# TACC/GraviT

Hardware: AMD Instinct MI355X
Metric: Mrays/s (primary+shadow) at 1080p, 10M-tri scene (higher is better)
Workload: dtype f32; 1 GPU; soup-10000000: 10000000 random triangles (Philox seed 12345, half-extent 0.005), 1920x1080, eye (.5,.5,3)->(.5,.5,.5), fov 30deg, 1 point light at the eye, depth 1 (primary + 1 shadow ray), AO off; scheduler=image, 1 domain, harness=native, settle_frames=0, normal_mode=flat

## Files before the change

### gravit_amd/capi.py

```python
import ctypes as C
import os

import numpy as np

from .layouts import HIT_DTYPE, LIGHT_DTYPE, MATERIAL_DTYPE, RAY_DTYPE

HERE = os.path.dirname(os.path.abspath(__file__))
LIB_PATH = os.environ.get("GVT_HIP_LIB") or os.path.join(HERE, "libgvt_hip.so")

ABI_VERSION = 6

SYMBOLS = [
    "gvt_hip_init", "gvt_hip_set_stream", "gvt_hip_synchronize", "gvt_hip_last_error",
    "gvt_hip_mesh_create", "gvt_hip_mesh_destroy", "gvt_hip_trace_ex", "gvt_hip_mesh_get_info", "gvt_hip_mesh_get_normals", "gvt_hip_mesh_update_vertices",
    "gvt_hip_trace", "gvt_hip_intersect", "gvt_hip_occluded",
    "gvt_hip_queue_create", "gvt_hip_queue_destroy", "gvt_hip_queue_reserve", "gvt_hip_queue_clear", "gvt_hip_queue_size",
    "gvt_hip_queue_append", "gvt_hip_queue_append_flags", "gvt_hip_abi_version", "gvt_hip_queue_export", "gvt_hip_trace_queue", "gvt_hip_trace_queue_sink",
    "gvt_hip_camera_generate",
    "gvt_hip_camera_generate_tiled",
    "gvt_hip_camera_filter",
    "gvt_hip_top_create", "gvt_hip_top_destroy", "gvt_hip_top_order", "gvt_hip_top_update", "gvt_hip_shuffle", "gvt_hip_queue_sizes",
    "gvt_hip_fb_create", "gvt_hip_fb_destroy", "gvt_hip_fb_clear", "gvt_hip_fb_download", "gvt_hip_fb_device_ptr",
    "gvt_hip_fb_write_ppm_bytes",
    "gvt_hip_profile", "gvt_hip_stats_read", "gvt_hip_stats_reset", "gvt_hip_set_option", "gvt_hip_is_experiments_build", "gvt_hip_counters_peek", "gvt_hip_visit_stats", "gvt_hip_wide_visit_stats", "gvt_hip_mesh_download_nodes", "gvt_hip_mesh_download_wide", "gvt_hip_mesh_download_clusters", "gvt_hip_mesh_upload_nodes", "gvt_hip_marked_visit_stats", "gvt_hip_image_frame",
# ... 8 lines not shown
    "gvt_hip_volume_create_typed", "gvt_hip_volume_update_samples_typed", "gvt_hip_volume_get_voxel_type",
]


class GvtHipError(RuntimeError):
    pass


class MeshInfo(C.Structure):
    _fields_ = [("n_tris", C.c_uint64), ("n_verts", C.c_uint64), ("n_nodes", C.c_uint64), ("n_leaves", C.c_uint64),
                ("bbox_lo", C.c_float * 3), ("bbox_hi", C.c_float * 3), ("build_ms", C.c_float), ("max_leaf", C.c_uint32),
                ("packet", C.c_uint32), ("bytes_nodes", C.c_uint64), ("bytes_tris", C.c_uint64), ("sah_inner", C.c_float), ("pad", C.c_float)]


class CameraPod(C.Structure):
    _fields_ = [("eye", C.c_float * 3), ("focus", C.c_float * 3), ("up", C.c_float * 3), ("fov", C.c_float), ("width", C.c_int32),
                ("height", C.c_int32), ("samples", C.c_int32), ("depth", C.c_int32), ("jitter_window_size", C.c_float)]


class FrameStats(C.Structure):
    _fields_ = [("rounds", C.c_uint64), ("chains", C.c_uint64), ("host_syncs", C.c_uint64), ("rays_sent", C.c_uint64),
                ("rays_closest", C.c_uint64), ("rays_any", C.c_uint64), ("packets_bailed", C.c_uint64), ("bytes_sent", C.c_uint64),
                ("ms_chain", C.c_double), ("ms_announce", C.c_double), ("ms_payload", C.c_double), ("ms_composite", C.c_double), ("ms_host_wait", C.c_double),
                ("exchanges", C.c_uint64), ("rays_inline", C.c_uint64)]

    def as_dict(self):
        return {k: getattr(self, k) for k, _ in self._fields_}


class VolumeInfo(C.Structure):
    _fields_ = [("box_lo", C.c_float * 3), ("box_hi", C.c_float * 3), ("dt", C.c_float), ("value_min", C.c_float), ("value_max", C.c_float),
                ("blocks", C.c_int32 * 3), ("pad", C.c_float), ("n_blocks", C.c_uint64), ("n_blocks_empty", C.c_uint64),
                ("samples_marched", C.c_uint64), ("samples_gathered", C.c_uint64)]

    def as_dict(self):
        return {k: (list(getattr(self, k)) if k in ("box_lo", "box_hi", "blocks") else getattr(self, k)) for k, _ in self._fields_ if k != "pad"}


RAY_OPAQUE, RAY_BOUNDARY, RAY_EXTERNAL_BOUNDARY = 0x2, 0x4, 0x10
RAY_SIDES = 0x20
VOLUME_MAX_SURFACES, VOLUME_MAX_LIGHTS = 16, 8
VOLUME_OPAQUE_A = 0.99
VOLUME_DEVICE, VOLUME_NO_SKIP = 1, 2
VOXEL_F32, VOXEL_U8, VOXEL_I16, VOXEL_U16 = 0, 1, 2, 3
VOXEL_TYPES = {"float32": VOXEL_F32, "uint8": VOXEL_U8, "int16": VOXEL_I16, "uint16": VOXEL_U16}

FRAME_BSP, FRAME_NO_COMPOSITE, FRAME_FULL_REDUCE, FRAME_IMAGE = 1, 2, 4, 8
# ... 113 lines not shown
```

### gravit_amd/csrc/api.hip

```cpp
#include <atomic>
#include <chrono>
#include <cmath>
#include <cstdlib>
#include <condition_variable>
#include <functional>
#include <mutex>
#include <new>
#include <thread>

#include "gvt_internal.h"

size_t trav_spill_ints_per_thread();
int trav_block_threads();
void abi_pool_destroy(void *);

static thread_local std::string g_err;
static Ctx g_default_ctx;
static thread_local Ctx *tl_ctx = nullptr;
#define g_ctx (gctx())
Ctx &gctx() { return tl_ctx ? *tl_ctx : g_default_ctx; }

void set_error(const char *fmt, ...) {
  char buf[1024];
  va_list ap;
// ... 191 lines not shown
extern "C" int gvt_hip_stats_reset(void) {
  if (ensure_init()) return GVT_HIP_ERR_NODEVICE;
  drain_events();
  g_ctx.stats = gvt_hip_stats{};
  return 0;
}

namespace {
struct KnobDef { const char *name; int Knobs::*field; int lo, hi; bool shipped; };
const KnobDef g_knobs[] = {
  { "skip_known", &Knobs::skip_known, 0, 1, true },           { "frame_timing", &Knobs::frame_timing, 0, 1, true },
  { "term_sink", &Knobs::term_sink, 0, 1, true },
  { "sort_rays", &Knobs::sort_rays, 0, 1, true },             { "leaf_max", &Knobs::leaf_max, 1, 4, true },
  { "long_steps", &Knobs::long_steps, 0, 1 << 20, true },     { "small_rays", &Knobs::small_rays, 0, 1 << 30, true },
  { "finish_rays", &Knobs::finish_rays, 0, 1 << 30, true },   { "round_room_mb", &Knobs::round_room_mb, 0, 1 << 30, true },
  { "abi_lanes", &Knobs::abi_lanes_n, 0, 8, true },           { "abi_chunk", &Knobs::abi_chunk, 16384, 1 << 30, true },
  { "inject_fail_tick", &Knobs::inject_fail_tick, -1, 1 << 30, true },
  { "long_min_rays", &Knobs::long_min_rays, 0, 1 << 30, true }, { "long_auto", &Knobs::long_auto, 0, 1, true },
  { "finish_auto", &Knobs::finish_auto, 0, 1, true },
  { "payload_overlap_kb", &Knobs::payload_overlap_kb, 0, 1 << 30, true },
  { "packet", &Knobs::packet, 0, 2, true },                   { "packet_sah_max", &Knobs::packet_sah_max, 0, 1 << 30, true },
  { "packet_min_rays", &Knobs::packet_min_rays, 0, 1 << 30, true },
  { "shadow_order", &Knobs::shadow_order, 0, 1, true },       { "shadow_order_min_rays", &Knobs::shadow_order_min_rays, 0, 1 << 30, true },
  { "xcd_stripes", &Knobs::xcd_stripes, 0, 1, true },

  { "inline_kb", &Knobs::inline_kb, 0, 1024, true },          { "comm_cus", &Knobs::comm_cus, 0, 128, true },
  { "comm_stream", &Knobs::comm_stream, 0, 1, true },         { "spec_ticks", &Knobs::spec_ticks, 0, 1, true },
  { "finish_clusters", &Knobs::finish_clusters, 0, 1, true }, { "hop_local", &Knobs::hop_local, 0, 3, true },
  { "blocks_per_cu", &Knobs::blocks_per_cu, 1, 8, false },    { "blocks_per_cu_closest", &Knobs::blocks_per_cu_closest, 0, 8, false },
  { "refill_min", &Knobs::refill_min, 1, 64, false },         { "inner_min", &Knobs::inner_min, 1, 64, false },
  { "share", &Knobs::share, 0, 1, false },                    { "share_min_rays", &Knobs::share_min_rays, 0, 1 << 30, false },
  { "sort_gather", &Knobs::sort_gather, 0, 1, false },        { "sort_bits", &Knobs::sort_bits, 8, 32, false },
  { "long_steps_drain", &Knobs::long_steps_drain, 0, 1 << 20, false }, { "long_save", &Knobs::long_save, 0, 1, false },
  { "lean_frame", &Knobs::lean_frame, 0, 1, false },          { "report_poll", &Knobs::report_poll, 0, 1, false },
  { "first_round_async", &Knobs::first_round_async, 0, 1, false }, { "wave_single", &Knobs::wave_single, 0, 1, false },
  { "shadow_direct", &Knobs::shadow_direct, 0, 1, false },    { "top_ordered", &Knobs::top_ordered, 0, 1, false },
  { "top_lds", &Knobs::top_lds, 0, 1, false },                { "camera_tile", &Knobs::camera_tile, 0, 8, false },
  { "abi_pipe_min", &Knobs::abi_pipe_min, 0, 1 << 30, false },
  { "shadow_cls_lo", &Knobs::shadow_cls_lo, 0, 255, false },  { "shadow_cls_shift", &Knobs::shadow_cls_shift, 0, 6, false },
};
}

extern "C" int gvt_hip_set_option(const char *name, int value) {
  if (!name) { set_error("set_option: null name"); return GVT_HIP_ERR_INVALID; }
  if (!std::strcmp(name, "defaults")) { static_cast<Knobs &>(g_ctx) = Knobs{}; return 0; }
  for (const KnobDef &k : g_knobs) {
    if (std::strcmp(name, k.name)) continue;
// ... 616 lines not shown
```

### gravit_amd/csrc/domain.hip

```cpp
#include <dlfcn.h>
#include <rccl/rccl.h>

#include <atomic>
#include <condition_variable>
#include <memory>
#include <mutex>

#include <chrono>
#include <thread>

#include "gvt_internal.h"

int shuffle_async(gvt_hip_top *T, gvt_hip_queue *q_in, size_t n_ub, const int *from_arr, int from, gvt_hip_queue *const *queues, const uint8_t *keep_mask,
                  gvt_hip_fb *fb, unsigned *d_overflow, const void *d_qdesc);
int shuffle_exact(gvt_hip_top *T, gvt_hip_queue *q_in, const int *from_arr, int from, gvt_hip_queue *const *queues, gvt_hip_fb *fb);
int camera_one_instance_async(gvt_hip_top *T, const gvt_hip_camera *cam, int tile, gvt_hip_queue *q, gvt_hip_fb *fb, unsigned *d_overflow, unsigned *d_moved_count, unsigned *row_rays);
int camera_filter_async(gvt_hip_top *T, const gvt_hip_camera *cam, int tile, gvt_hip_queue *const *queues, const uint8_t *keep_mask, unsigned *d_overflow,
                        size_t first, size_t count, bool rect = false, unsigned *row_rays = nullptr);
size_t camera_instance_bound(gvt_hip_top *T, const gvt_hip_camera *cam, int tile, size_t inst);

namespace {
struct Rccl {
  void *lib = nullptr;
  ncclResult_t (*GetUniqueId)(ncclUniqueId *) = nullptr;
// ... 716 lines not shown
  size_t inl_bytes = 0, msg_ints = 0;
  double tick_us[8] = { 0 }; uint64_t tick_n[8] = { 0 }; double comp_us = 0;
  uint64_t n_spec_enqueued = 0, n_spec_valid = 0, n_exchanges = 0;
  size_t spec_recent_rays = 0;
  bool sizes_exact = true;
  bool spec_enqueued_last = false;
  unsigned *d_spec = nullptr;
  WaveSeg *d_spec_segs = nullptr;
  bool layout_agreed = false;
  int *d_hs = nullptr, *h_hs = nullptr;
  unsigned *d_overflow = nullptr;
  std::vector<void *> send_buf, recv_buf;
  std::vector<size_t> send_cap, recv_cap;
  hipEvent_t ev_compute = nullptr, ev_report = nullptr, ev_pack = nullptr, ev_recv = nullptr, ev_comm = nullptr;
  hipEvent_t ev_chain0 = nullptr, ev_ann0 = nullptr, ev_pay0 = nullptr, ev_comp0 = nullptr;
  bool chain_timed = false, payload_timed = false;
  uint64_t last_local_pending = 0;
  std::vector<size_t> present;
  int long_cur = 0;
  uint64_t frame_no = 0;
  int fin_choice = -1;
  int fin_limit = 0;
  int hop_now = 0;
  unsigned cam_row_rays = 0;
  bool fin_eligible = false;
  unsigned fin_probe = 0;
  double fin_best[6] = { 1e30, 1e30, 1e30, 1e30, 1e30, 1e30 };
  int fin_n[6] = { 0, 0, 0, 0, 0, 0 };
  bool surfaces = false;
};

extern "C" void gvt_hip_tracer_destroy(gvt_hip_tracer *R) {
  if (!R) return;
  if (getenv("GVT_HIP_SPEC_TRACE") && R->n_exchanges)
    fprintf(stderr, "[tracer rank %d] %llu announce exchanges, speculative part enqueued behind %llu, valid %llu\n", R->rank, (unsigned long long)R->n_exchanges,
            (unsigned long long)R->n_spec_enqueued, (unsigned long long)R->n_spec_valid);
  if (getenv("GVT_HIP_SPEC_TRACE") && R->tick_n[0]) {
    fprintf(stderr, "[tracer rank %d] mean us from frame start / previous announce to the announce of tick:", R->rank);
    for (int k = 0; k < 8 && R->tick_n[k]; k++) fprintf(stderr, " %d: %.1f", k, R->tick_us[k] / (double)R->tick_n[k]);
    fprintf(stderr, "; last announce to frame end %.1f\n", R->comp_us / (double)R->tick_n[0]);
  }
  if (gctx().ready) hipStreamSynchronize(gctx().stream);
  if (R->comm && !R->comm->dead) hipStreamSynchronize(R->comm->stream);
  for (auto q : R->queues) gvt_hip_queue_destroy(q);
  gvt_hip_queue_destroy(R->q_moved);
  hipFree(R->d_insts); hipFree(R->d_round); hipHostFree(R->h_round); hipFree(R->d_count_ptr); hipFree(R->d_owner);
// ... 211 lines not shown
  R->sizes_exact = false;
  for (int k = 0; k < n_seg; k++) {
    gvt_hip_queue *q = R->queues[R->h_segs[k].inst];
    R->h_segs[k].planes = q->d_planes; R->h_segs[k].cap = q->cap;
  }
  hipStream_t st = C.stream;
  for (size_t i = 0; i < nI; i++) {
    gvt_hip_queue *Q = R->queues[i];
    R->h_qdesc[i].planes = Q->d_planes; R->h_qdesc[i].cap = Q->cap; R->h_qdesc[i].count = Q->d_count; R->h_qdesc[i].keep = 1u;
  }
  for (size_t k = (size_t)n_seg; k < (nI ? nI : 1); k++) std::memset(&R->h_segs[k], 0, sizeof(WaveSeg));
  if ((rc = round_tables_upload(R, st))) return rc;
  int *d_from = (int *)scratch_get(SCR_OUT_FROM, sizeof(int) * bound);
  if (!d_from) return GVT_HIP_ERR_DEVICE;
  TraceParams P{};
  P.normal_mode = R->normal_mode; P.seed = 0; P.n_lights = nL; P.update_in_place = 0; P.carried_rng = 1;
  P.sink = TermSink{};
  if (C.term_sink) {
    P.sink.top = R->top->dev(); P.sink.from = -1;
    P.sink.fb = R->fb->d_rgba; P.sink.n_pix = (unsigned)(R->fb->w * R->fb->h);
  }
  P.hop = R->hop_now == 1 ? 1 : R->hop_now == 2 ? 2 : 0;
  P.hop_owner = R->world > 1 ? R->d_owner : nullptr; P.hop_rank = R->rank;
  WaveSet W{ R->d_segs, R->d_insts, n_seg, (int)nI };
  if (C.finish_rays > 0 && N <= (size_t)C.finish_rays && P.sink.fb && !count_on_device && !exact) R->fin_eligible = true;
  if (R->fin_limit > 0 && N <= (size_t)R->fin_limit && P.sink.fb && !count_on_device && !exact) {
    if ((rc = finish_round(W, N, P, R->lights.data(), R->d_qdesc, R->d_owner, R->world > 1 ? R->rank : -1, R->d_overflow, R->d_count_ptr, R->d_mask))) return rc;
    if (chains) (*chains)++;
    return 0;
  }
  WaveSingle one{};
  if (n_seg == 1 && R->meshes[R->h_segs[0].inst] && C.wave_single && !P.hop) {
    const int i0 = R->h_segs[0].inst;
    one.planes = make_planes(R->h_segs[0].planes, R->h_segs[0].cap);
    if (nI == 1) one.planes.p5 = nullptr;
    one.mesh = R->meshes[i0]; one.inst = i0;
    one.coherent = (fresh_from_camera && C.camera_tile == 8) ? 1 : 0;
    one.row_rays = one.coherent ? R->cam_row_rays : 0u;
    one.n_dev = count_on_device ? R->queues[i0]->d_count : nullptr;
    one.pass0_begun = pass0_begun ? 1 : 0;
    std::memcpy(one.minv.m, R->minv.data() + 16 * (size_t)i0, 64);
    std::memcpy(one.normi.n, R->normi.data() + 9 * (size_t)i0, 36);
  }
  const bool single = one.mesh != nullptr;
  ChainOpts O;
  O.d_count_ptr = R->d_count_ptr; O.d_mask = R->d_mask; O.n_inst = (int)nI;
// ... 226 lines not shown
    if ((R->frame_no & 2047u) == 0 || (R->fin_choice >= 0 && !((allowed >> R->fin_choice) & 1u))) {
      R->fin_choice = -1;
      for (int v = 0; v < 6; v++) { R->fin_n[v] = 0; R->fin_best[v] = 1e30; }
    }
    if (R->fin_choice >= 0) fin_variant = R->fin_choice;
    else {
      int pick = fin_variant;
      for (int k = 0; k < n_allowed; k++) if (R->fin_n[route_list[k]] < R->fin_n[pick]) pick = route_list[k];
      fin_variant = pick;
    }
  }
  R->fin_limit = (fin_variant & 1) ? C.finish_rays : 0;
  R->hop_now = fin_variant >> 1;
  R->fin_eligible = false;
  struct LongOverride { Ctx &C; ~LongOverride() { C.long_steps_override = 0; } } long_override{ C };
  C.long_steps_override = (C.long_auto && C.long_steps > 0 && R->long_cur > C.long_steps) ? R->long_cur : 0;
  const bool one_shot = nI == 1 && R->world == 1 && C.term_sink && C.wave_single && R->meshes[0] && C.first_round_async;
  const bool lean = one_shot && C.lean_frame && R->fb->w == R->cam.width && R->fb->h == R->cam.height;
  for (size_t i = 0; i < nI; i++) R->queues[i]->size = 0;
  R->q_moved->size = 0;
  R->sizes_exact = true; R->spec_enqueued_last = false;
  R->cam_row_rays = 0u;
  bool first_on_device = false;
  if (!lean) {
    if ((rc = gvt_hip_fb_clear(R->fb))) return rc;
    k_zero_totals<<<(unsigned)std::max<size_t>(1, (nI + 255) / 256), 256, 0, st>>>(C.d_counters, R->d_overflow, R->fb->w, R->fb->h, R->d_count_ptr, (int)nI);
  }
  if (one_shot) {
    const size_t n_cam = (size_t)R->cam.width * R->cam.height * R->cam.samples * R->cam.samples;
    const int passes0 = R->cam.depth > 1 ? R->cam.depth : 1;
    if ((rc = queue_reserve(R->queues[0], n_cam * (size_t)(1 + (int)R->lights.size() * passes0)))) return rc;
    if (lean) { if ((rc = camera_one_instance_async(R->top, &R->cam, C.camera_tile, R->queues[0], R->fb, R->d_overflow, R->q_moved->d_count, &R->cam_row_rays))) return rc; }
    else if ((rc = camera_filter_async(R->top, &R->cam, C.camera_tile, R->queues.data(), nullptr, R->d_overflow, 0, 0, false, &R->cam_row_rays))) return rc;
    R->present[0] = n_cam;
    R->queues[0]->size = n_cam;
    if ((rc = local_chain(R, nullptr, &S.chains, true, true, lean, lean))) return rc;
    if ((rc = round_report(R, false, &S.host_syncs, lean))) return rc;
  } else if (image_split) {
    const size_t n_cam = (size_t)R->cam.width * R->cam.height * R->cam.samples * R->cam.samples;
    const size_t portion = n_cam / (size_t)R->world, first = (size_t)R->rank * portion;
    const size_t count = (R->rank + 1 == R->world) ? n_cam - first : portion;
    for (size_t i = 0; i < nI; i++) if ((rc = queue_reserve(R->queues[i], count))) return rc;
    if ((rc = camera_filter_async(R->top, &R->cam, C.camera_tile, R->queues.data(), nullptr, R->d_overflow, first, count))) return rc;
    std::fill(R->owned.begin(), R->owned.end(), (uint8_t)1);
    R->world = 1;
    if ((rc = round_report(R, false, &S.host_syncs))) return rc;
// ... 281 lines not shown
    R->fin_n[fin_variant]++;
    R->fin_probe++;
    bool once = true;
    double lead = 1e30;
    for (int k = 0; k < n_allowed; k++) { once = once && R->fin_n[route_list[k]] >= 1; lead = std::min(lead, R->fin_best[route_list[k]]); }
    if (once) for (int k = 0; k < n_allowed; k++) if (R->fin_best[route_list[k]] > 1.3 * lead) R->fin_n[route_list[k]] = std::max(R->fin_n[route_list[k]], 3);
    bool all = true;
    int best = route_list[0];
    for (int k = 0; k < n_allowed; k++) {
      all = all && R->fin_n[route_list[k]] >= 3;
      if (R->fin_best[route_list[k]] < R->fin_best[best] || (R->fin_best[route_list[k]] == R->fin_best[best] && route_list[k] > best)) best = route_list[k];
    }
    if (all) {
      R->fin_choice = best;
      if (getenv("GVT_HIP_ROUTE_TRACE")) {
        fprintf(stderr, "[tracer] frame %llu: route settled -- k_finish %d, hops %s; fastest frame per route timed, ms:", (unsigned long long)R->frame_no, best & 1,
                (best >> 1) == 0 ? "never" : (best >> 1) == 1 ? "early" : "always");
        for (int k = 0; k < n_allowed; k++) fprintf(stderr, " [k_finish %d hops %d] %.3f", route_list[k] & 1, route_list[k] >> 1, R->fin_best[route_list[k]]);
        fprintf(stderr, "\n");
      }
    }
  }
  R->frame_no++;
  if (out) *out = S;
  return 0;
}
```

### gravit_amd/csrc/gvt_internal.h

```cpp
#pragma once
#include <hip/hip_runtime.h>

#include <cstdarg>
#include <cstdio>
#include <cstring>
#include <string>
#include <vector>

#include "gvt_device.h"

enum KernelClass { KC_CLOSEST = 0, KC_ANY, KC_SHADE, KC_CONVERT, KC_SHUFFLE, KC_CAMERA, KC_BUILD, KC_SORT, KC_LONG, KC_COUNT };

struct PendingEvent {
  hipEvent_t a, b;
  int cls;
};

#define SHADOW_CLASSES 8
static_assert(CW_SHADOW_CLS + SHADOW_CLASSES <= CW_PEEK, "the class counts are read through gvt_hip_counters_peek");
static_assert(CW_SHADOW_CLS + SHADOW_CLASSES <= CW_COUNT && CW_PEEK <= CW_COUNT, "every named counter word lies inside the allocation");

enum ScratchSlot {
  SCR_GENERAL,
  SCR_SHADOW,
// ... 13 lines not shown
  SCR_VOL_RANGES,
  SCR_BUILD,
  SCR_HOP,
  SCRATCH_COUNT
};
struct Knobs {
  int blocks_per_cu = 4;
  int blocks_per_cu_closest = 5;
  int refill_min = 16;
  int inner_min = 32;
  int share = 1;
  int share_min_rays = 131072;
  int sort_rays = 0;
  int sort_gather = 0;
  int sort_bits = 20;
  int long_steps = 96;
  int long_steps_drain = 0;
  int long_save = 1;
  int long_min_rays = 65536;
  int packet = 1;
  int shadow_order = 1;
  int shadow_cls_lo = 24, shadow_cls_shift = 3;
  int xcd_stripes = 1;
  int shadow_order_min_rays = 262144;
  int packet_min_rays = 524288;
  int packet_sah_max = 128;
  int round_room_mb = 16384;
  int finish_rays = 32768;
  int finish_auto = 1;
  int small_rays = 4096;
  int abi_lanes_n = 4;
  int abi_chunk = 262144;
  int abi_pipe_min = 131072;
  int lean_frame = 1;
  int skip_known = 0;
  int long_auto = 1;
  int payload_overlap_kb = 1024;
  int inline_kb = 16;
  int comm_cus = 0;
  int hop_local = 1;
  int finish_clusters = 1;
  int spec_ticks = 1;
  int comm_stream = 0;
  int frame_timing = 0;
  int inject_fail_tick = -1;
  int report_poll = 1;
  int first_round_async = 1;
  int wave_single = 1;
  int shadow_direct = 1;
  int term_sink = 1;
  int camera_tile = 8;
  int top_ordered = 1;
  int top_lds = 1;
  int leaf_max = 2;
};

struct Ctx : Knobs {
  bool ready = false;
  int device = -1;
  hipStream_t own_stream = nullptr;
  hipStream_t stream = nullptr;
  int profile = 0;
  int long_steps_override = 0;
  std::vector<PendingEvent> pending;
  std::vector<hipEvent_t> event_pool;
  gvt_hip_stats stats{};
  int n_cu = 256;
  bool shadow_order_denied = false;
  int cu_reserved = 0;
  int trav_blocks = 0;
  int *d_spill = nullptr;
  unsigned *d_counters = nullptr;
  unsigned *h_pinned = nullptr;
  void *scratch[SCRATCH_COUNT] = { nullptr };
  size_t scratch_bytes[SCRATCH_COUNT] = { 0 };
  std::vector<unsigned char> lights_cached;
  const void *lights_cached_dst = nullptr;
  gvt_hip_queue *abi_qin = nullptr, *abi_qout = nullptr;
  std::vector<Ctx *> abi_lanes;
  void *abi_pool = nullptr;
};
Ctx &gctx();
void set_error(const char *fmt, ...);
int ensure_init();
inline bool staging_queues(Ctx &C) {
  if (!C.abi_qin) { C.abi_qin = gvt_hip_queue_create(0); C.abi_qout = gvt_hip_queue_create(0); }
  return C.abi_qin && C.abi_qout;
}
void *scratch_get(ScratchSlot slot, size_t bytes);
void scratch_release(ScratchSlot slot);
// ... 78 lines not shown
  unsigned long long cap;
  unsigned *count;
  unsigned keep;
};

struct TermSink {
  TopDev top;
  int from;
  float *fb;
  unsigned n_pix;
};
struct TraceParams {
  Mat4 m, minv;
  Mat3 normi;
  int normal_mode;
  uint32_t seed;
  int n_lights;
  TermSink sink;
  int update_in_place;
  int carried_rng;
  int hop;
  const int *hop_owner;
  int hop_rank;
};

struct MeshView {
  const float4 *slots;
  const unsigned *slot_of;
  const float *verts;
  const int *tris;
  const float *normals;
  const float *vcolors;
  const gvt_hip_material *materials;
  unsigned n_mat;
  const int *face_mat;
  gvt_hip_material mat;
};

struct WaveSeg {
  float4 *planes;
  unsigned long long cap;
  unsigned begin, n;
  int inst, pad;
};
struct WaveInst {
  Mat4 minv;
// ... 67 lines not shown
```

### gravit_amd/csrc/shade.inc

```
__device__ inline V3 light_contribution(const gvt_hip_light &L, V3 hit, V3 samplePos) {
  V3 c = ld3(L.color);
  if (L.type == GVT_HIP_LIGHT_AMBIENT) return c;
  V3 p = (L.type == GVT_HIP_LIGHT_AREA) ? samplePos : ld3(L.position);
  float distance = 1.f / len3(sub3(p, hit));
  distance = (distance > 1.f) ? 1.f : distance;
  return scl3(c, distance);
}

__device__ inline V3 area_light_position(const gvt_hip_light &L, uint32_t &seed) {
  V3 v = ld3(L.normal), u, w;
  if (v.x == 0.f && v.y == 1.f && v.z == 0.f) {
    u = mk3(1, 0, 0); w = mk3(0, 0, 1);
  } else {
    const V3 up = mk3(0, 1, 0);
    u.x = up.y * v.z - v.y * up.z; u.y = up.z * v.x - v.z * up.x; u.z = up.x * v.y - v.x * up.y;
    w.x = v.y * u.z - u.y * v.z; w.y = v.z * u.x - u.z * v.x; w.z = v.x * u.y - u.x * v.y;
  }
  float xLocation = (float)(((double)gvt_fastrand_lcg(seed, 0, 1) - 0.5) * (double)L.width);
  float zLocation = (float)(((double)gvt_fastrand_lcg(seed, 0, 1) - 0.5) * (double)L.height);
  float xCoord = xLocation * u.x + zLocation * w.x;
  float yCoord = xLocation * u.y + zLocation * w.y;
  float zCoord = xLocation * u.z + zLocation * w.z;
  return mk3(L.position[0] + xCoord, L.position[1] + yCoord, L.position[2] + zCoord);
}
// ... 123 lines not shown
  const gvt_hip_hit *hits;
  int first_pass;
  int carried_rng;
  RayPlanes out; unsigned *out_count;
  RayPlanes shadow; unsigned *shadow_count;
  unsigned *next_idx; unsigned *next_count;
  const gvt_hip_light *lights;
  Mat3 normi;
  int normal_mode, n_lights;
  uint32_t seed;
  unsigned *zero_word;
  TermSink sink;
  int update_in_place;
  const unsigned *n_dev;
  WaveSet W;
  const int *hop_inst;
  int *out_from;
  int *shadow_inst;
  unsigned shadow_stride;
  const unsigned char *steps;
  unsigned *cls_cnt;
  unsigned cls_stride;
  int cls_lo, cls_shift;
};

__device__ __forceinline__ unsigned shadow_class(int steps, int lo, int shift) {
  const int c = (steps - lo) >> shift;
  return (unsigned)(c < 0 ? 0 : (c > SHADOW_CLASSES - 1 ? SHADOW_CLASSES - 1 : c));
}

#define SHADE_BLOCK 512
template <bool MULTI, bool LEAN = false>
__global__ __launch_bounds__(SHADE_BLOCK, 4) void k_shade(ShadeArgs A, MeshView M1) {
  __shared__ unsigned sh_alloc[2 * (2 + 64)];
  __shared__ unsigned sh_cls[2 * SHADOW_CLASSES];
  for (int k = threadIdx.x; k < 2 * (2 + 64); k += SHADE_BLOCK) sh_alloc[k] = 0u;
  if (threadIdx.x < 2 * SHADOW_CLASSES) sh_cls[threadIdx.x] = 0u;
  __syncthreads();
  const unsigned j = blockIdx.x * blockDim.x + threadIdx.x;
  if (j == 0 && A.zero_word) *A.zero_word = 0u;
  const unsigned n = A.n_dev ? *A.n_dev : A.n;
  const bool in_range = j < n;
  __shared__ unsigned sh_wcls[SHADE_BLOCK / 64];
  if (!MULTI && A.cls_cnt) {
    int st = in_range ? (int)A.steps[j] : 0;
    for (int o = 32; o >= 1; o >>= 1) st = max(st, __shfl_xor(st, o));
    if (lane_id() == 0) sh_wcls[threadIdx.x >> 6] = shadow_class(st, A.cls_lo, A.cls_shift);
// ... 91 lines not shown
        s.c = c; s.t = r.t;
        s.id = r.id; s.depth = r.depth; s.w = r.w; s.type = 1;
        s.rng = 0u;
        s.km[0] = 0u; s.km[1] = 0u; s.km[2] = 0u;
      }
    }
    if (A.shadow_stride) {
      if (j < A.shadow_stride) {
        const unsigned slot = (unsigned)li * A.shadow_stride + j;
        A.shadow_inst[slot] = emit ? (MULTI ? inst : 0) : -1;
        if (emit) store_ray(A.shadow, slot, s);
      }
    } else if (!MULTI && A.cls_cnt) {
      const unsigned cls = (unsigned)__builtin_amdgcn_readfirstlane((int)sh_wcls[threadIdx.x >> 6]);
      const unsigned long long mask = ballot64(emit);
      unsigned woff = 0;
      if (mask) {
        if ((int)lane_id() == __ffsll((long long)mask) - 1) woff = atomicAdd(&sh_cls[cls], (unsigned)__popcll(mask));
        woff = (unsigned)__builtin_amdgcn_readlane((int)woff, __ffsll((long long)mask) - 1);
      }
      __syncthreads();
      if (threadIdx.x < SHADOW_CLASSES && sh_cls[threadIdx.x]) sh_cls[SHADOW_CLASSES + threadIdx.x] = atomicAdd(&A.cls_cnt[threadIdx.x], sh_cls[threadIdx.x]);
      __syncthreads();
      if (emit) store_ray(A.shadow, cls * A.cls_stride + sh_cls[SHADOW_CLASSES + cls] + woff + lanes_below(mask), s);
    } else {
      const unsigned slot = block_alloc(A.shadow_count, emit, &sh_alloc[2 * (2 + li)]);
      if (emit) { store_ray(A.shadow, slot, s); if (MULTI) A.shadow_inst[slot] = inst; }
    }
  }
  if (!LEAN && shaded) {
    const int ndepth = r.depth - 1;
    const float p = 1.f - gvt_fastrand01(g_seed);
    if (ndepth > 0 && r.w > p) {
      r.type = 2;
      const float multiplier = 1.0f - 16.0f * GVT_FLT_EPSILON;
      const float t_secondary = multiplier * r.t;
      r.o = add3(r.o, scl3(r.d, t_secondary));
      const V3 nd = cos_weighted_dir(N, g_seed);
      r.d = nd;
      r.w = r.w * dot3(nd, N);
      r.depth = ndepth;
      r.km[0] = 0u; r.km[1] = 0u; r.km[2] = 0u;
      bounce = true;
    }
    if (bounce || A.update_in_place) {
      r.rng = g_seed;
      store_ray(in, i, r);
    }
  }
  if (!LEAN) {
// ... 5 lines not shown
```

### gravit_amd/csrc/trace.hip

```cpp
#include "gvt_internal.h"

#ifndef TRAV_BLOCK
#define TRAV_BLOCK 256
#endif
#define TRAV_WAVES_PER_BLOCK (TRAV_BLOCK / 64)
#ifndef TRAV_STACK
#define TRAV_STACK 24
#endif
#ifndef KT_BLOCKS_CLOSEST
#define KT_BLOCKS_CLOSEST 5
#endif
#ifndef RETIRE_BATCH
#define RETIRE_BATCH 1
#endif
#ifndef KT_BLOCKS_ANY
#define KT_BLOCKS_ANY 4
#endif
#define TRAV_SPILL 128

namespace {

struct Trav {
  const BvhNode *__restrict__ nodes;
  const float4 *__restrict__ tris;
// ... 193 lines not shown
    ProfScope ps(KC_CLOSEST);
    LongQ LP{ d_long, c + CW_LONG, nullptr, 0u, 0, 0 };
    if constexpr (MULTI) k_packet_multi<<<blocks_for(n), 256, 0, st>>>(S.W, (unsigned)n, n_dev, tnear, d_hits, LP, c + CW_PACKETS);
    else k_packet<false><<<blocks_for(n), 256, 0, st>>>(S.q, (unsigned)n, n_dev, S.minv, S.T, tnear, d_hits, nullptr, none, nullptr, TermSink{}, LP, nullptr, nullptr, nullptr, c + CW_PACKETS);
    k_long_closest<XFORM, MULTI><<<tail_grid, 256, 0, st>>>(S.q, d_long, c + CW_LONG, S.minv, S.T, tnear, d_hits, c + CW_LONG_WORK, S.W);
  } else if (mode == BY_WAVES) {
    ProfScope ps(KC_CLOSEST);
    k_long_seed<<<blocks_for(n), 256, 0, st>>>(d_long, c + CW_LONG, idx, (unsigned)n, n_dev);
    k_long_closest<XFORM, MULTI><<<wave_grid(n), 256, 0, st>>>(S.q, d_long, c + CW_LONG, S.minv, S.T, tnear, d_hits, c + CW_LONG_WORK, S.W, nullptr, later_pass ? S.hop : nullptr);
  } else {
    {
      ProfScope ps(KC_CLOSEST);
      launch_trace<false, XFORM, 0, MULTI>(trav_grid2(n, true), st, S.q, idx, (unsigned)n, S.minv, S.T, tnear, d_hits, nullptr, none, nullptr, c + CW_WORK, C.d_spill,
                                           C.refill_min, C.inner_min, n_dev, C.share, (unsigned)C.share_min_rays, S.sink, LQ, S.MS, MULTI ? XCD_STRIPES_OFF : stripe_arg(S.row));
    }
    if (LQ.steps) {
      ProfScope ps(KC_LONG);
      k_long_closest<XFORM, MULTI><<<tail_grid, 256, 0, st>>>(S.q, LQ.recs, LQ.count, S.minv, S.T, tnear, d_hits, c + CW_LONG_WORK, S.W, LQ.stk, S.hop);
    }
  }
}

template <bool MULTI>
static void any_step(StepMode mode, const TraceSrc &S, const unsigned *idx, size_t grid_rays, unsigned n, const unsigned *n_dev, RayPlanes out, unsigned *out_count) {
  Ctx &C = gctx();
  unsigned *c = C.d_counters;
  ProfScope ps(KC_ANY);
  if (mode == BY_WAVES) k_wave_any<MULTI><<<wave_grid(grid_rays), 256, 0, C.stream>>>(S.q, c + CW_SHADOW, S.minv, S.T, GVT_RAY_EPSILON, out, out_count, c + CW_WORK, S.sink, S.MS);
  else launch_trace<true, true, 1, MULTI>(trav_grid2(grid_rays), C.stream, S.q, idx, n, S.minv, S.T, GVT_RAY_EPSILON, nullptr, nullptr, out, out_count, c + CW_WORK, C.d_spill,
                                          C.refill_min, C.inner_min, n_dev, C.share, (unsigned)C.share_min_rays, S.sink, LongQ{}, S.MS, MULTI ? XCD_STRIPES_OFF : stripe_arg(S.row));
}

static ShadeArgs shade_args(const ChainBufs &B, const unsigned *idx, size_t n, int pass, const unsigned *n_dev, unsigned *next, unsigned *c_next, RayPlanes outp,
                            unsigned *out_count, const TraceParams &P) {
  unsigned *c = gctx().d_counters;
  ShadeArgs A{};
  A.idx = idx; A.n = (unsigned)n; A.hits = B.hits; A.first_pass = (pass == 0); A.carried_rng = 1; A.out = outp; A.out_count = out_count;
  A.shadow = B.shadow; A.shadow_count = c + CW_SHADOW; A.next_idx = next; A.next_count = c_next; A.lights = B.lights; A.normi = P.normi; A.normal_mode = P.normal_mode;
  A.n_lights = P.n_lights; A.seed = P.seed; A.zero_word = c + CW_WORK; A.sink = P.sink; A.n_dev = n_dev;
  return A;
}

template <bool MULTI>
static void shade_step(const ShadeArgs &A, const MeshView &mv, bool lean = false) {
  ProfScope ps(KC_SHADE);
  if (lean) k_shade<MULTI, true><<<blocks_for(A.n, SHADE_BLOCK), SHADE_BLOCK, 0, gctx().stream>>>(A, mv);
  else k_shade<MULTI><<<blocks_for(A.n, SHADE_BLOCK), SHADE_BLOCK, 0, gctx().stream>>>(A, mv);
}

int launch_closest(gvt_hip_mesh *M, RayPlanes q, const unsigned *idx, size_t n, bool xform, const Mat4 &minv, float tnear,
// ... 199 lines not shown
  Ctx &C = gctx();
  unsigned *c = C.d_counters;
  gvt_hip_mesh *M = W1.mesh;
  const size_t n = K.n;
  const int nL = K.P.n_lights;
  const bool have4 = M->d_nodes4 != nullptr, by_class = K.B.steps != nullptr;
  if (C.sort_rays && p.pass > 0 && n >= 8192 && have4)
    if (int rc = sort_ray_list(M, W1.planes, &p.idx, n, n, W1.minv, p.n_dev)) return rc;
  TraceSrc S{};
  S.q = W1.planes; S.minv = W1.minv; S.T = Trav{ M->d_nodes, M->d_tri, M->d_nodes4 };
  S.row = (W1.coherent && p.pass == 0 && !p.idx) ? W1.row_rays : 0u;
  LongQ LQ{};
  if (K.use_long && have4) LQ = long_queue(K.d_long, n);
  LQ.steps_out = K.B.steps;
  const bool small1 = K.small && have4;
  const bool pkt = walks_packets(C, M, n) && W1.coherent && p.pass == 0 && have4 && !small1;
  const bool pkt_any = pkt && C.packet == 2;
  closest_step<true, false>(pkt ? BY_PACKETS : small1 ? BY_WAVES : BY_LANES, S, p.idx, n, p.n_dev, GVT_RAY_EPSILON, K.B.hits, LQ, K.d_long);
  ShadeArgs A = shade_args(K.B, p.idx, n, p.pass, p.n_dev, p.next, p.c_next, K.outp, K.out->d_count, K.P);
  A.in = W1.planes; A.normi = W1.normi; A.sink.from = W1.inst;
  if (pkt_any) { A.shadow_inst = K.d_shadow_inst; A.shadow_stride = (unsigned)n; }
  A.steps = K.B.steps; A.cls_cnt = by_class ? c + CW_SHADOW_CLS : nullptr; A.cls_stride = (unsigned)cls_stride; A.cls_lo = C.shadow_cls_lo; A.cls_shift = C.shadow_cls_shift;
  const bool lean_shade = W1.coherent && p.pass == 0 && K.passes == 1 && K.P.sink.fb && K.P.sink.top.n_inst == 1 && nL >= 1 && plain_lambert(M) && no_area_light(K.lights_host, nL);
  shade_step<false>(A, mesh_view(M), lean_shade);
  if (!nL) return 0;
  TraceSrc SA = S;
  SA.q = K.B.shadow; SA.sink = A.sink; SA.row = 0u;
  if (pkt_any) return any_packets(K, SA);
  if (by_class) { SA.MS.cls_cnt = c + CW_SHADOW_CLS; SA.MS.cls_stride = (unsigned)cls_stride; SA.MS.cls_total = c + CW_SHADOW; }
  any_step<false>(small1 ? BY_WAVES : BY_LANES, SA, nullptr, K.B.shadow_cap, 0u, by_class ? nullptr : c + CW_SHADOW, K.outp, K.out->d_count);
  return 0;
}

static void merged_pass(const Chain &K, const Pass &p, const WaveSet &W, const ChainOpts &O, int *d_hop, int *d_out_from) {
  Ctx &C = gctx();
  unsigned *c = C.d_counters;
  const TraceParams &P = K.P;
  const size_t n = K.n;
  const int nL = P.n_lights;
  TraceSrc S{};
  S.W = W; S.MS.W = W; S.hop = d_hop;
  if (d_hop) {
    S.sink = P.sink;
    S.MS.hop_inst = d_hop; S.MS.hop_read = p.pass > 0; S.MS.hop_owner = P.hop_owner; S.MS.hop_rank = P.hop_rank; S.MS.hop_tot = cw_totals(c) + TOT_CLOSEST; S.MS.hop_early = P.hop == 1 ? 1 : 0;
  }
  LongQ LQ{};
  if (K.use_long) LQ = long_queue(K.d_long, n);
  const bool pktm = O.multi_packets && p.pass == 0 && !K.small && p.idx == nullptr;
  closest_step<true, true>(pktm ? BY_PACKETS : K.small ? BY_WAVES : BY_LANES, S, p.idx, n, p.n_dev, GVT_RAY_EPSILON, K.B.hits, LQ, K.d_long, p.pass > 0);
  ShadeArgs A = shade_args(K.B, p.idx, n, p.pass, p.n_dev, p.next, p.c_next, K.outp, K.out->d_count, P);
  A.W = W; A.out_from = d_out_from; A.shadow_inst = K.d_shadow_inst; A.hop_inst = d_hop;
  const bool direct = C.shadow_direct && p.pass == 0 && !K.small;
  const bool direct_dev = direct && K.nd0 != nullptr && nL == 1;
// ... 90 lines not shown
```

### gravit_amd/csrc/trace_lane.inc

```
#ifndef GVT_TRI_NG_FROM_SLOT
#define GVT_TRI_NG_FROM_SLOT 1
#endif
#ifndef GVT_STAMP
#define GVT_STAMP 0
#endif
#if GVT_STAMP
__device__ unsigned long long g_stamp[24];
#endif
#ifndef TRAV_CHUNK
#define TRAV_CHUNK 256
#endif
#ifndef KT_SHARE_DELAY
#define KT_SHARE_DELAY 24
#endif
#define TRAV_DONE ((int)0x80000000)

#define LONG_SAVE 48
#define LONG_STK_CAP 65536u
struct LongRec { unsigned j, i; float bt; int bp; float bu, bv, bden; unsigned ns; };
struct LongQ {
  LongRec *recs;
  unsigned *count;
  int *stk;
  unsigned stk_cap;
// ... 322 lines not shown
            } else {
              const WaveSeg sg = MS.W.segs[wave_find_seg(MS.W, i)];
              const unsigned local = i - sg.begin;
              a = sg.planes[local]; b = sg.planes[sg.cap + local];
              inst_l = sg.inst; gidx = i;
              if (MS.hop_read) { const int h_ = MS.hop_inst[i]; if (h_ >= 0) inst_l = h_; }
            }
            if (start && tab) {
              nodes4_l = s_inst[inst_l].nodes4; tris_l = s_inst[inst_l].tris;
              O = xfm_point(s_inst[inst_l].minv, mk3(a.x, a.y, a.z)); D = xfm_vector(s_inst[inst_l].minv, mk3(b.x, b.y, b.z));
            } else if (start) {
              const WaveInst *wi = MS.W.insts + inst_l;
              nodes4_l = wi->nodes4; tris_l = wi->tris;
              O = xfm_point(wi->minv, mk3(a.x, a.y, a.z)); D = xfm_vector(wi->minv, mk3(b.x, b.y, b.z));
            }
          } else {
            a = q.p0[i]; b = q.p1[i];
            O = mk3(a.x, a.y, a.z); D = mk3(b.x, b.y, b.z);
            if (XFORM) {
              const float *m = minv.m;
              O = xfm_point(minv, O);
              D = mk3((m[0] * D.x + m[4] * D.y) + (m[8] * D.z + z12), (m[1] * D.x + m[5] * D.y) + (m[9] * D.z + z13), (m[2] * D.x + m[6] * D.y) + (m[10] * D.z + z14));
            }
            if (ANY && MODE == 1) j = i;
          }
          if (start) {
            const float dx = fabsf(D.x) < 1e-30f ? copysignf(1e-30f, D.x) : D.x;
            const float dy = fabsf(D.y) < 1e-30f ? copysignf(1e-30f, D.y) : D.y;
            const float dz = fabsf(D.z) < 1e-30f ? copysignf(1e-30f, D.z) : D.z;
            const float ix = 1.0f / dx, iy = 1.0f / dy, iz = 1.0f / dz;
            S = make_slab(ix, iy, iz, O.x * ix, O.y * iy, O.z * iz);
            bt = GVT_FLT_MAX; bu = 0.f; bv = 0.f; bden = 1.f; bp = -1;
            sp = 0; sb = 0; nsteps = 0;
            cur = (MULTI ? nodes4_l : T.nodes4) != nullptr ? 0 : TRAV_DONE;
            active = true;
          }
        }
        if (MULTI && ANY) n_started += (unsigned)__popcll(ballot64(start));
        c_next += take;
        idle = ballot64(!active);
        nidle = __popcll(idle);
      }
    }
    if (nidle == 64) break;
    const bool share_on = ANY && (share & 1) != 0;
    if (exhausted) drain_iters++;
    const bool share_now = share_on && exhausted && drain_iters > KT_SHARE_DELAY && n >= share_min;
// ... 6 lines not shown
        const int sbd = __shfl(sb, d);
        const unsigned gj = (unsigned)__shfl((int)j, d);
        const float gOx = __shfl(O.x, d), gOy = __shfl(O.y, d), gOz = __shfl(O.z, d);
        const float gDx = __shfl(D.x, d), gDy = __shfl(D.y, d), gDz = __shfl(D.z, d);
        RaySlab gS;
        gS.ix = __shfl(S.ix, d); gS.iy = __shfl(S.iy, d); gS.iz = __shfl(S.iz, d);
        gS.ox = (f2){ __shfl(S.ox.x, d), __shfl(S.ox.y, d) }; gS.oy = (f2){ __shfl(S.oy.x, d), __shfl(S.oy.y, d) }; gS.oz = (f2){ __shfl(S.oz.x, d), __shfl(S.oz.y, d) };
        const int gbp = __shfl(bp, d);
        const int ginst = __shfl(inst_l, d);
        if ((int)lane_id() == h) {
          if (MULTI) { inst_l = ginst; nodes4_l = MS.W.insts[ginst].nodes4; tris_l = MS.W.insts[ginst].tris; }
          const unsigned tid_d = wave_tid0 + (unsigned)d;
          cur = (sbd < TRAV_STACK) ? stack[sbd * TRAV_BLOCK + tid_d]
                                   : spill_base[((size_t)blockIdx.x * TRAV_BLOCK + tid_d) * TRAV_SPILL + (sbd - TRAV_STACK)];
          j = gj; O = mk3(gOx, gOy, gOz); D = mk3(gDx, gDy, gDz);
          S = gS; bp = gbp;
          sp = 0; sb = 0;
          active = true;
        }
        if ((int)lane_id() == d) sb++;
        idle_m &= idle_m - 1;
        don_m &= don_m - 1;
        sharing = true;
      }
    }
#if GVT_STAMP == 1
    { unsigned long long t_ = __builtin_amdgcn_s_memtime(); st_refill += t_ - t_mark; t_mark = t_; n_outer_it++; }
#endif
    unsigned long long im = ballot64(cur >= 0);
    const float lim2 = fminf(cull_bound(bt), 3.40282326e38f);
    while (im) {
      const bool at_inner = cur >= 0;
      if (at_inner) {
        float tn[4];
        int rr[4];
        bool entered[4];
        node4_test<ANY>((const uint4 *)((const char *)(MULTI ? nodes4_l : T.nodes4) + ((unsigned)cur << 6)), S, GVT_FLT_MAX, tn, rr, ANY ? entered : nullptr);
#define KT_ENTERED(K) (ANY ? entered[K] : (tn[K] <= lim2))
        if (!ANY) sort4(tn, rr);
        int nxt = TRAV_DONE;
        bool have = false;
        if (sp + 3 <= TRAV_STACK) {
#pragma unroll
          for (int c4 = 3; c4 >= 0; c4--) {
            if (KT_ENTERED(c4)) {
              if (have) { lds[sp * TRAV_BLOCK] = nxt; sp++; }
// ... 140 lines not shown
        n_pend += __popcll(sm);
      }
      if (n_pend >= 64) { flush_pending(pend, n_pend, q, out, out_count, sink, MULTI ? MS.ray_inst : nullptr, MULTI ? MS.out_from : nullptr); n_pend = 0; }
    }
    if (!ANY && LQ.steps) {
      const unsigned long long pm = ballot64(fin && KT_PARKED);
      if (pm) {
        unsigned base = 0;
        if ((int)lane_id() == __ffsll((long long)pm) - 1) base = atomicAdd(LQ.count, (unsigned)__popcll(pm));
        base = __shfl(base, __ffsll((long long)pm) - 1);
        if (fin && KT_PARKED) {
          const unsigned slot = base + lanes_below(pm);
          LongRec R; R.j = j; R.i = MULTI ? gidx : (idx ? idx[j] : j); R.bt = bt; R.bp = bp; R.bu = bu; R.bv = bv; R.bden = bden; R.ns = 0u;
          const int depth = sp - sb;
          if (LQ.stk && depth > 0 && depth <= LONG_SAVE && slot < LQ.stk_cap) {
            int *dst = LQ.stk + (size_t)slot * LONG_SAVE;
            for (int k = 0; k < depth; k++) dst[k] = (sb + k < TRAV_STACK) ? lds[(sb + k) * TRAV_BLOCK] : KT_SPILL(sb + k - TRAV_STACK);
            R.ns = (unsigned)depth;
          }
          LQ.recs[slot] = R;
        }
      }
    }
    if (fin) {
      if (ANY) { if (MODE == 0) flags[j] = (bp >= 0) ? 1 : 0; }
      else {
        if (!KT_PARKED) { gvt_hip_hit h; h.t = bt; h.prim = bp; h.u = (bp >= 0) ? bu / bden : 0.f; h.v = (bp >= 0) ? bv / bden : 0.f; hits[j] = h; }
        if (LQ.steps_out) LQ.steps_out[j] = (unsigned char)(KT_PARKED ? 255 : min(nsteps, 254));
      }
      active = false;
    }
  }
#if GVT_STAMP
  if (lane_id() == 0) { atomicAdd(&g_stamp[0], st_refill); atomicAdd(&g_stamp[1], st_inner); atomicAdd(&g_stamp[2], st_leaf); atomicAdd(&g_stamp[3], st_retire); atomicAdd(&g_stamp[4], n_inner_it); atomicAdd(&g_stamp[5], n_outer_it); atomicAdd(&g_stamp[6], 1ull); atomicAdd(&g_stamp[7], (unsigned long long)__builtin_amdgcn_s_memtime() - t_begin); atomicAdd(&g_stamp[14], n_inner_lanes); atomicAdd(&g_stamp[15], n_leaf_lanes); atomicMax(&g_stamp[16], ~t_begin); atomicMax(&g_stamp[17], (unsigned long long)__builtin_amdgcn_s_memtime()); atomicMax(&g_stamp[18], t_exh); atomicAdd(&g_stamp[19], t_exh ? t_exh - t_begin : 0ull); atomicMax(&g_stamp[20], (unsigned long long)__builtin_amdgcn_s_memtime() - t_begin); atomicMax(&g_stamp[21], t_exh ? t_exh - t_begin : 0ull); atomicMax(&g_stamp[22], ~(t_exh ? t_exh - t_begin : ~0ull));
    if (t_exh) { atomicAdd(&g_stamp[8], (unsigned long long)__builtin_amdgcn_s_memtime() - t_exh); atomicAdd(&g_stamp[9], n_inner_it - it_exh); atomicAdd(&g_stamp[10], n_outer_it - out_exh); atomicAdd(&g_stamp[11], act_exh); atomicMax(&g_stamp[12], (unsigned long long)__builtin_amdgcn_s_memtime() - t_exh); atomicMax(&g_stamp[13], n_inner_it - it_exh); } }
#endif
  if (ANY && MODE == 1) { if (n_pend) flush_pending(pend, n_pend, q, out, out_count, sink, MULTI ? MS.ray_inst : nullptr, MULTI ? MS.out_from : nullptr); }
  if (MULTI && ANY && MS.tot_any && n_started && lane_id() == 0) atomicAdd(MS.tot_any, (unsigned long long)n_started);
  if (MULTI && MS.hop_tot && n_hops && lane_id() == 0) atomicAdd(MS.hop_tot, (unsigned long long)n_hops);
#undef KT_PUSH
#undef KT_POP
#undef KT_SPILL
#undef KT_PARKED
}
```

### include/gvt_hip.h

```cpp
#ifndef GVT_HIP_H
#define GVT_HIP_H

#include <stddef.h>
#include <stdint.h>

#ifdef __cplusplus
extern "C" {
#endif

#define GVT_HIP_ABI_VERSION 6
int gvt_hip_abi_version(void);

#define GVT_HIP_OK 0
#define GVT_HIP_ERR_INVALID (-1)
#define GVT_HIP_ERR_DEVICE (-2)
#define GVT_HIP_ERR_CAPACITY (-3)
#define GVT_HIP_ERR_NODEVICE (-4)
#define GVT_HIP_ERR_TIMEOUT (-5)
#define GVT_HIP_ERR_PEER (-6)

#define GVT_HIP_NORMALS_FLAT 0
#define GVT_HIP_NORMALS_SMOOTH 1

typedef struct gvt_hip_ray {
// ... 152 lines not shown
int gvt_hip_tracer_set_camera(gvt_hip_tracer *, const gvt_hip_camera *cam);
int gvt_hip_tracer_set_transforms(gvt_hip_tracer *, const float *m , const float *minv, const float *normi , size_t n_inst);
int gvt_hip_tracer_set_domains(gvt_hip_tracer *, const int32_t *owner , gvt_hip_comm *comm);
#define GVT_HIP_FRAME_BSP 1
#define GVT_HIP_FRAME_NO_COMPOSITE 2
#define GVT_HIP_FRAME_IMAGE 8
#define GVT_HIP_FRAME_FULL_REDUCE 4
typedef struct gvt_hip_frame_stats {
  uint64_t rounds;
  uint64_t chains;
  uint64_t host_syncs;
  uint64_t rays_sent;
  uint64_t rays_closest;
  uint64_t rays_any;
  uint64_t packets_bailed;
  uint64_t bytes_sent;
  double ms_chain;
  double ms_announce;
  double ms_payload;
  double ms_composite;
  double ms_host_wait;
  uint64_t exchanges;
  uint64_t rays_inline;
} gvt_hip_frame_stats;
int gvt_hip_tracer_frame(gvt_hip_tracer *, int flags, gvt_hip_frame_stats *stats);

#define GVT_HIP_RAY_OPAQUE 0x2
#define GVT_HIP_RAY_BOUNDARY 0x4
#define GVT_HIP_RAY_EXTERNAL_BOUNDARY 0x10
#define GVT_HIP_VOLUME_OPAQUE_A 0.99f
#define GVT_HIP_VOLUME_DEVICE 1
#define GVT_HIP_VOLUME_NO_SKIP 2
typedef struct gvt_hip_volume gvt_hip_volume;
gvt_hip_volume *gvt_hip_volume_create(const float *samples, const int counts[3], const float origin[3], const float spacing[3], const int offset[3],
                                      const int global_counts[3], float sampling_rate, int flags);
void gvt_hip_volume_destroy(gvt_hip_volume *);
typedef struct gvt_hip_volume_info {
  float box_lo[3], box_hi[3];
  float dt;
  float value_min, value_max;
  int32_t blocks[3];
  float pad;
  uint64_t n_blocks, n_blocks_empty;
  uint64_t samples_marched;
  uint64_t samples_gathered;
} gvt_hip_volume_info;
// ... 61 lines not shown
```

Measured before the change: 2407 Mrays/s.

## Deposit shadow contributions optimistically at shade time and clear on occlusion

```diff
diff --git a/gravit_amd/capi.py b/gravit_amd/capi.py
--- a/gravit_amd/capi.py
+++ b/gravit_amd/capi.py
@@ -54,7 +54,7 @@
     _fields_ = [("rounds", C.c_uint64), ("chains", C.c_uint64), ("host_syncs", C.c_uint64), ("rays_sent", C.c_uint64),
                 ("rays_closest", C.c_uint64), ("rays_any", C.c_uint64), ("packets_bailed", C.c_uint64), ("bytes_sent", C.c_uint64),
                 ("ms_chain", C.c_double), ("ms_announce", C.c_double), ("ms_payload", C.c_double), ("ms_composite", C.c_double), ("ms_host_wait", C.c_double),
-                ("exchanges", C.c_uint64), ("rays_inline", C.c_uint64)]
+                ("exchanges", C.c_uint64), ("rays_inline", C.c_uint64), ("early_deposit_launches", C.c_uint64)]
 
     def as_dict(self):
         return {k: getattr(self, k) for k, _ in self._fields_}
diff --git a/gravit_amd/csrc/api.hip b/gravit_amd/csrc/api.hip
--- a/gravit_amd/csrc/api.hip
+++ b/gravit_amd/csrc/api.hip
@@ -237,7 +237,7 @@
   { "packet", &Knobs::packet, 0, 2, true },                   { "packet_sah_max", &Knobs::packet_sah_max, 0, 1 << 30, true },
   { "packet_min_rays", &Knobs::packet_min_rays, 0, 1 << 30, true },
   { "shadow_order", &Knobs::shadow_order, 0, 1, true },       { "shadow_order_min_rays", &Knobs::shadow_order_min_rays, 0, 1 << 30, true },
-  { "xcd_stripes", &Knobs::xcd_stripes, 0, 1, true },
+  { "xcd_stripes", &Knobs::xcd_stripes, 0, 1, true },           { "early_deposit", &Knobs::early_deposit, 0, 1, true },
 
   { "inline_kb", &Knobs::inline_kb, 0, 1024, true },          { "comm_cus", &Knobs::comm_cus, 0, 128, true },
   { "comm_stream", &Knobs::comm_stream, 0, 1, true },         { "spec_ticks", &Knobs::spec_ticks, 0, 1, true },
diff --git a/gravit_amd/csrc/domain.hip b/gravit_amd/csrc/domain.hip
--- a/gravit_amd/csrc/domain.hip
+++ b/gravit_amd/csrc/domain.hip
@@ -762,6 +762,7 @@
   int fin_choice = -1;
   int fin_limit = 0;
   int hop_now = 0;
+  bool fb_fresh = false;
   unsigned cam_row_rays = 0;
   bool fin_eligible = false;
   unsigned fin_probe = 0;
@@ -1019,6 +1020,8 @@
   }
   P.hop = R->hop_now == 1 ? 1 : R->hop_now == 2 ? 2 : 0;
   P.hop_owner = R->world > 1 ? R->d_owner : nullptr; P.hop_rank = R->rank;
+  P.one_writer = (fresh_from_camera && R->fb_fresh && R->cam.samples == 1) ? 1 : 0;
+  R->fb_fresh = false;
   WaveSet W{ R->d_segs, R->d_insts, n_seg, (int)nI };
   if (C.finish_rays > 0 && N <= (size_t)C.finish_rays && P.sink.fb && !count_on_device && !exact) R->fin_eligible = true;
   if (R->fin_limit > 0 && N <= (size_t)R->fin_limit && P.sink.fb && !count_on_device && !exact) {
@@ -1291,6 +1294,8 @@
   R->sizes_exact = true; R->spec_enqueued_last = false;
   R->cam_row_rays = 0u;
   bool first_on_device = false;
+  R->fb_fresh = true;
+  const uint64_t early0 = C.early_deposit_launches;
   if (!lean) {
     if ((rc = gvt_hip_fb_clear(R->fb))) return rc;
     k_zero_totals<<<(unsigned)std::max<size_t>(1, (nI + 255) / 256), 256, 0, st>>>(C.d_counters, R->d_overflow, R->fb->w, R->fb->h, R->d_count_ptr, (int)nI);
@@ -1618,6 +1623,7 @@
     }
   }
   R->frame_no++;
+  S.early_deposit_launches = C.early_deposit_launches - early0;
   if (out) *out = S;
   return 0;
 }
diff --git a/gravit_amd/csrc/gvt_internal.h b/gravit_amd/csrc/gvt_internal.h
--- a/gravit_amd/csrc/gvt_internal.h
+++ b/gravit_amd/csrc/gvt_internal.h
@@ -59,6 +59,7 @@
   int shadow_order = 1;
   int shadow_cls_lo = 24, shadow_cls_shift = 3;
   int xcd_stripes = 1;
+  int early_deposit = 1;
   int shadow_order_min_rays = 262144;
   int packet_min_rays = 524288;
   int packet_sah_max = 128;
@@ -103,6 +104,7 @@
   std::vector<hipEvent_t> event_pool;
   gvt_hip_stats stats{};
   int n_cu = 256;
+  uint64_t early_deposit_launches = 0;
   bool shadow_order_denied = false;
   int cu_reserved = 0;
   int trav_blocks = 0;
@@ -227,6 +229,7 @@
   int hop;
   const int *hop_owner;
   int hop_rank;
+  int one_writer;
 };
 
 struct MeshView {
diff --git a/gravit_amd/csrc/shade.inc b/gravit_amd/csrc/shade.inc
--- a/gravit_amd/csrc/shade.inc
+++ b/gravit_amd/csrc/shade.inc
@@ -169,7 +169,19 @@
   unsigned *cls_cnt;
   unsigned cls_stride;
   int cls_lo, cls_shift;
+  int early_deposit;
 };
+
+__device__ __forceinline__ void store_shadow_early(const ShadeArgs &A, unsigned slot, const RayRec &s) {
+  A.shadow.p0[slot] = make_float4(s.o.x, s.o.y, s.o.z, s.t_min);
+  A.shadow.p1[slot] = make_float4(s.d.x, s.d.y, s.d.z, s.t_max);
+  const bool dep = len3(s.c) > 0.f && (unsigned)s.id < A.sink.n_pix;
+  if (dep) {
+    const V3 cw = scl3(s.c, s.w);
+    ((float4 *)A.sink.fb)[(unsigned)s.id] = make_float4(0.0f + cw.x, 0.0f + cw.y, 0.0f + cw.z, 1.0f);
+  }
+  ((uint32_t *)A.shadow.p2)[slot] = dep ? (uint32_t)s.id : 0xffffffffu;
+}
 
 __device__ __forceinline__ unsigned shadow_class(int steps, int lo, int shift) {
   const int c = (steps - lo) >> shift;
@@ -307,10 +319,18 @@
       __syncthreads();
       if (threadIdx.x < SHADOW_CLASSES && sh_cls[threadIdx.x]) sh_cls[SHADOW_CLASSES + threadIdx.x] = atomicAdd(&A.cls_cnt[threadIdx.x], sh_cls[threadIdx.x]);
       __syncthreads();
-      if (emit) store_ray(A.shadow, cls * A.cls_stride + sh_cls[SHADOW_CLASSES + cls] + woff + lanes_below(mask), s);
+      if (emit) {
+        const unsigned slot = cls * A.cls_stride + sh_cls[SHADOW_CLASSES + cls] + woff + lanes_below(mask);
+        if (LEAN && A.early_deposit) store_shadow_early(A, slot, s);
+        else store_ray(A.shadow, slot, s);
+      }
     } else {
       const unsigned slot = block_alloc(A.shadow_count, emit, &sh_alloc[2 * (2 + li)]);
-      if (emit) { store_ray(A.shadow, slot, s); if (MULTI) A.shadow_inst[slot] = inst; }
+      if (emit) {
+        if (LEAN && !MULTI && A.early_deposit) store_shadow_early(A, slot, s);
+        else store_ray(A.shadow, slot, s);
+        if (MULTI) A.shadow_inst[slot] = inst;
+      }
     }
   }
   if (!LEAN && shaded) {
diff --git a/gravit_amd/csrc/trace.hip b/gravit_amd/csrc/trace.hip
--- a/gravit_amd/csrc/trace.hip
+++ b/gravit_amd/csrc/trace.hip
@@ -239,10 +239,18 @@
 }
 
 template <bool MULTI>
-static void any_step(StepMode mode, const TraceSrc &S, const unsigned *idx, size_t grid_rays, unsigned n, const unsigned *n_dev, RayPlanes out, unsigned *out_count) {
+static void any_step(StepMode mode, const TraceSrc &S, const unsigned *idx, size_t grid_rays, unsigned n, const unsigned *n_dev, RayPlanes out, unsigned *out_count, bool early = false) {
   Ctx &C = gctx();
   unsigned *c = C.d_counters;
   ProfScope ps(KC_ANY);
+  if constexpr (!MULTI) {
+    if (early && mode == BY_LANES) {
+      launch_trace<true, true, 2, false>(trav_grid2(grid_rays), C.stream, S.q, idx, n, S.minv, S.T, GVT_RAY_EPSILON, nullptr, nullptr, out, out_count, c + CW_WORK, C.d_spill,
+                                         C.refill_min, C.inner_min, n_dev, C.share, (unsigned)C.share_min_rays, S.sink, LongQ{}, S.MS, stripe_arg(S.row));
+      C.early_deposit_launches++;
+      return;
+    }
+  }
   if (mode == BY_WAVES) k_wave_any<MULTI><<<wave_grid(grid_rays), 256, 0, C.stream>>>(S.q, c + CW_SHADOW, S.minv, S.T, GVT_RAY_EPSILON, out, out_count, c + CW_WORK, S.sink, S.MS);
   else launch_trace<true, true, 1, MULTI>(trav_grid2(grid_rays), C.stream, S.q, idx, n, S.minv, S.T, GVT_RAY_EPSILON, nullptr, nullptr, out, out_count, c + CW_WORK, C.d_spill,
                                           C.refill_min, C.inner_min, n_dev, C.share, (unsigned)C.share_min_rays, S.sink, LongQ{}, S.MS, MULTI ? XCD_STRIPES_OFF : stripe_arg(S.row));
@@ -488,13 +496,15 @@
   if (pkt_any) { A.shadow_inst = K.d_shadow_inst; A.shadow_stride = (unsigned)n; }
   A.steps = K.B.steps; A.cls_cnt = by_class ? c + CW_SHADOW_CLS : nullptr; A.cls_stride = (unsigned)cls_stride; A.cls_lo = C.shadow_cls_lo; A.cls_shift = C.shadow_cls_shift;
   const bool lean_shade = W1.coherent && p.pass == 0 && K.passes == 1 && K.P.sink.fb && K.P.sink.top.n_inst == 1 && nL >= 1 && plain_lambert(M) && no_area_light(K.lights_host, nL);
+  const bool early_deposit = lean_shade && nL == 1 && K.P.one_writer && !small1 && !pkt_any && C.early_deposit;
+  A.early_deposit = early_deposit ? 1 : 0;
   shade_step<false>(A, mesh_view(M), lean_shade);
   if (!nL) return 0;
   TraceSrc SA = S;
   SA.q = K.B.shadow; SA.sink = A.sink; SA.row = 0u;
   if (pkt_any) return any_packets(K, SA);
   if (by_class) { SA.MS.cls_cnt = c + CW_SHADOW_CLS; SA.MS.cls_stride = (unsigned)cls_stride; SA.MS.cls_total = c + CW_SHADOW; }
-  any_step<false>(small1 ? BY_WAVES : BY_LANES, SA, nullptr, K.B.shadow_cap, 0u, by_class ? nullptr : c + CW_SHADOW, K.outp, K.out->d_count);
+  any_step<false>(small1 ? BY_WAVES : BY_LANES, SA, nullptr, K.B.shadow_cap, 0u, by_class ? nullptr : c + CW_SHADOW, K.outp, K.out->d_count, early_deposit);
   return 0;
 }
 
diff --git a/gravit_amd/csrc/trace_lane.inc b/gravit_amd/csrc/trace_lane.inc
--- a/gravit_amd/csrc/trace_lane.inc
+++ b/gravit_amd/csrc/trace_lane.inc
@@ -368,7 +368,7 @@
               O = xfm_point(minv, O);
               D = mk3((m[0] * D.x + m[4] * D.y) + (m[8] * D.z + z12), (m[1] * D.x + m[5] * D.y) + (m[9] * D.z + z13), (m[2] * D.x + m[6] * D.y) + (m[10] * D.z + z14));
             }
-            if (ANY && MODE == 1) j = i;
+            if (ANY && MODE >= 1) j = i;
           }
           if (start) {
             const float dx = fabsf(D.x) < 1e-30f ? copysignf(1e-30f, D.x) : D.x;
@@ -421,6 +421,9 @@
         idle_m &= idle_m - 1;
         don_m &= don_m - 1;
         sharing = true;
+#if GVT_STAMP
+        if (lane_id() == 0) atomicAdd(&g_stamp[23], 1ull);
+#endif
       }
     }
 #if GVT_STAMP == 1
@@ -607,6 +610,12 @@
         }
       }
     }
+    if (ANY && MODE == 2) {
+      if (fin && bp >= 0) {
+        const unsigned px = ((const unsigned *)q.p2)[j];
+        if (px != 0xffffffffu) ((float4 *)sink.fb)[px] = make_float4(0.f, 0.f, 0.f, 0.f);
+      }
+    }
     if (fin) {
       if (ANY) { if (MODE == 0) flags[j] = (bp >= 0) ? 1 : 0; }
       else {
diff --git a/include/gvt_hip.h b/include/gvt_hip.h
--- a/include/gvt_hip.h
+++ b/include/gvt_hip.h
@@ -198,6 +198,7 @@
   double ms_host_wait;
   uint64_t exchanges;
   uint64_t rays_inline;
+  uint64_t early_deposit_launches;
 } gvt_hip_frame_stats;
 int gvt_hip_tracer_frame(gvt_hip_tracer *, int flags, gvt_hip_frame_stats *stats);
 
```

After: 2501 Mrays/s, median of 6. 3.9% higher.
